# stonkgs/stonkgs

Measured on AMD Instinct MI355X. Metric: text-triple pairs/sec (whole node), seq_len=512 hidden=768, 1/2/4/8 MI355X, higher is better.
Workload: dtype bf16; 1 GPU; STonKGs-150k pretraining step (12L/768h, V=28996, K=175094), per-GPU batch 64, seq 256 text + 256 entity, dropout 0.1, AdamW lr 1e-4; global_batch=64, seq_len=512, parallelism=dp1

## Files before the change

### include/stonk_hip.h

```cpp
#ifndef STONK_HIP_H
#define STONK_HIP_H
#include <stdint.h>
#include "../stonkgs_amd/csrc/stonk_flags.h"

#ifdef __cplusplus
extern "C" {
#endif

#define STONK_OK 0
#define STONK_EINVAL (-1)
#define STONK_ESHAPE (-2)
#define STONK_EALIGN (-3)

int stonk_abi_version(void);

int stonk_gemm_nt_bf16(const void* A, int64_t lda, const void* B, int64_t ldb, void* C, int64_t ldc, int M, int N, int K,
                       int flags, const float* bias, const void* resid, int64_t ldr, void* aux, int64_t ldaux,
                       float alpha, int split_k, const int* m_dev, const int* k_dev, float drop_p, uint32_t seed,
                       int kernel, void* stream);

int stonk_gemm_tn_bf16(const void* dY, int64_t lda, const void* X, int64_t ldb, float* dW, int64_t ldc, float* dbias,
                       int M, int N, int K, float alpha, int split_k, const int* k_dev, void* stream);
int stonk_gemm_tn_bf16_store(const void* dY, int64_t lda, const void* X, int64_t ldb, float* dW, int64_t ldc, float* dbias,
                             int M, int N, int K, float alpha, int split_k, const int* k_dev, void* stream);
int stonk_gemm_tn_bf16_store_sumsq(const void* dY, int64_t lda, const void* X, int64_t ldb, float* dW, int64_t ldc,
                                   float* dbias, int M, int N, int K, float alpha, int split_k, const int* k_dev,
                                   float* tile_sumsq, int64_t n_slots, void* stream);
int64_t stonk_gemm_tn_store_tiles(int M, int N, int K, int split_k);

int stonk_layernorm_fwd(const void* x, const float* gamma, const float* beta, void* y, float* mean, float* rstd,
                        int64_t rows, int H, float eps, int flags, float drop_p, uint32_t seed, void* stream);

int64_t stonk_layernorm_bwd_workspace_floats(int64_t rows, int H);
int stonk_layernorm_bwd(const void* dy, const void* x, const float* mean, const float* rstd, const float* gamma,
                        void* dx, void* dx_drop, float* dgamma, float* dbeta, int64_t rows, int H, int flags,
                        float drop_p_in, uint32_t seed_in, float drop_p_out, uint32_t seed_out, float* partial_ws,
                        int64_t ws_floats, void* stream);
int stonk_layernorm_bwd_reduce(const float* partial_ws, int64_t rows, int H, float* dgamma, float* dbeta, void* stream);

int stonk_joint_embed_ln_fwd(const int64_t* input_ids, const int64_t* token_type_ids, const void* text_hidden,
                             const float* kg_table, const float* pos_emb, const float* type_emb, const float* gamma,
                             const float* beta, void* sum_out, void* y, float* mean, float* rstd, int B, int S,
                             int half, int H, int64_t kg_rows, int type_rows, float eps, int flags, float drop_p,
                             uint32_t seed, int* err_flag, const int* pos_of_row, int64_t n_rows, void* stream);

int stonk_text_embed_ln_fwd(const int64_t* input_ids, int64_t ld_ids, const float* word_emb, const float* pos_emb,
                            const float* type_emb, const float* gamma, const float* beta, void* y, int B, int S, int H,
                            int64_t vocab, float eps, int flags, float drop_p, uint32_t seed, int* err_flag,
                            void* stream);

int stonk_embed_grad(const void* dx, const int64_t* token_type_ids, float* dpos, float* dtype, int B, int S, int H,
                     int type_rows, const int* row_of_pos, void* stream);

int stonk_word_embed_grad(const void* dsum, int64_t ld, const int64_t* input_ids, const int* row_of_pos, float* dword,
                          int64_t ld_w, int64_t vocab, int padding_idx, int B, int S, int H, int* err_flag, void* stream);
// ... 155 lines not shown
```

### stonkgs_amd/_hip.py

```python
from __future__ import annotations

import ctypes as C
import os

_HERE = os.path.dirname(os.path.abspath(__file__))
LIB_PATH = os.environ.get("STONK_HIP_LIB") or os.path.join(_HERE, "csrc", "libstonk_hip.so")

EPI_OUT_BF16 = 0
EPI_OUT_F32 = 1
EPI_OUT_F32_ATOMIC = 2
EPI_OUT_F16 = 3
EPI_BIAS = 1 << 2
EPI_GELU = 1 << 3
EPI_RESID = 1 << 4
EPI_SAVE_PREACT = 1 << 5
EPI_GELU_BWD = 1 << 6
EPI_DROPOUT = 1 << 7
EPI_AUX_GRAD = 1 << 8
GEMM_AUTO, GEMM_TILE128, GEMM_WAVE8, GEMM_WAVE4, GEMM_WAVE4_192, GEMM_DISPATCHED, GEMM_DISPATCHED2 = 0, 1, 2, 3, 4, 5, 6
GEMM_ASM4, GEMM_ASM4_192 = 7, 8
LN_DROPOUT = 1 << 0
LN_DEFER_REDUCE = 1 << 1
SMALL_TANH = 1
SMALL_X_F32 = 16
LOSS_MSE, LOSS_MSE_BROADCAST, LOSS_BCE = 0, 1, 2
OK, EINVAL, ESHAPE, EALIGN = 0, -1, -2, -3
ATTN_BWD_DELTA, ATTN_BWD_DQ, ATTN_BWD_DKV, ATTN_BWD_ALL = 1, 2, 4, 7

_vp, _i32, _i64, _f32, _u32, _f64 = C.c_void_p, C.c_int, C.c_int64, C.c_float, C.c_uint32, C.c_double

_SIGNATURES = {
    "stonk_gemm_nt_bf16": [_vp, _i64, _vp, _i64, _vp, _i64, _i32, _i32, _i32, _i32, _vp, _vp, _i64, _vp, _i64,
                           _f32, _i32, _vp, _vp, _f32, _u32, _i32, _vp],
    "stonk_gemm_tn_bf16": [_vp, _i64, _vp, _i64, _vp, _i64, _vp, _i32, _i32, _i32, _f32, _i32, _vp, _vp],
    "stonk_gemm_tn_bf16_store": [_vp, _i64, _vp, _i64, _vp, _i64, _vp, _i32, _i32, _i32, _f32, _i32, _vp, _vp],
    "stonk_gemm_tn_bf16_store_sumsq": [_vp, _i64, _vp, _i64, _vp, _i64, _vp, _i32, _i32, _i32, _f32, _i32, _vp, _vp, _i64, _vp],
    "stonk_layernorm_fwd": [_vp, _vp, _vp, _vp, _vp, _vp, _i64, _i32, _f32, _i32, _f32, _u32, _vp],
    "stonk_layernorm_bwd": [_vp, _vp, _vp, _vp, _vp, _vp, _vp, _vp, _vp, _i64, _i32, _i32, _f32, _u32, _f32, _u32,
                            _vp, _i64, _vp],
    "stonk_layernorm_bwd_reduce": [_vp, _i64, _i32, _vp, _vp, _vp],
    "stonk_joint_embed_ln_fwd": [_vp, _vp, _vp, _vp, _vp, _vp, _vp, _vp, _vp, _vp, _vp, _vp, _i32, _i32, _i32, _i32,
                                 _i64, _i32, _f32, _i32, _f32, _u32, _vp, _vp, _i64, _vp],
    "stonk_unpad_plan": [_vp, _vp, _vp, _i32, _i32, _i32, _vp, _vp, _vp, _vp, _vp, _vp, _vp, _vp, _i64, _vp],
    "stonk_text_embed_ln_fwd": [_vp, _i64, _vp, _vp, _vp, _vp, _vp, _vp, _i32, _i32, _i32, _i64, _f32, _i32, _f32,
                                _u32, _vp, _vp],
    "stonk_embed_grad": [_vp, _vp, _vp, _vp, _i32, _i32, _i32, _i32, _vp, _vp],
    "stonk_word_embed_grad": [_vp, _i64, _vp, _vp, _vp, _i64, _i64, _i32, _i32, _i32, _i32, _vp, _vp],
    "stonk_input_attribution": [_vp, _i64, _vp, _vp, _vp, _i64, _vp, _f32, _vp, _vp, _vp, _i64, _i32, _i32, _i32, _i32, _vp],
    "stonk_attention_fwd": [_vp, _vp, _vp, _i64, _vp, _vp, _vp, _vp, _i64, _vp, _i32, _i32, _i32, _i32, _f32, _f32, _u32, _vp],
    "stonk_attention_bwd": [_vp, _vp, _vp, _i64, _vp, _vp, _vp, _vp, _i64, _vp, _i64, _vp, _vp, _vp, _vp, _i64, _vp, _i32,
                            _i32, _i32, _i32, _f32, _f32, _u32, _vp],
    "stonk_attention_bwd_phases": [_i32, _vp, _vp, _vp, _i64, _vp, _vp, _vp, _vp, _i64, _vp, _i64, _vp, _vp, _vp, _vp, _i64, _vp,
                                   _i32, _i32, _i32, _i32, _f32, _f32, _u32, _vp],
    "stonk_block_sparse_attention_fwd": [_vp, _vp, _vp, _i64, _vp, _vp, _vp, _vp, _vp, _i64, _vp, _i32, _i32, _i32, _i32, _f32,
                                         _vp, _vp],
    "stonk_block_sparse_attention_bwd": [_vp, _vp, _vp, _i64, _vp, _vp, _vp, _vp, _vp, _vp, _vp, _vp, _i64, _vp, _i64, _vp, _vp,
                                         _vp, _vp, _i64, _vp, _i32, _i32, _i32, _i32, _f32, _vp, _vp],
    "stonk_attention_probs": [_vp, _vp, _i64, _vp, _vp, _vp, _i32, _i32, _i32, _i32, _i32, _f32, _vp],
    "stonk_transpose_bf16": [_vp, _i64, _vp, _i64, _i64, _i32, _vp, _vp, _vp],
    "stonk_transpose_f32_to_bf16": [_vp, _vp, _i64, _i32, _i64, _vp],
    "stonk_transpose_bf16_batched": [_vp, _i32, _i32, _vp],
    "stonk_cast_f32_to_bf16": [_vp, _vp, _i64, _vp],
    "stonk_mlm_mask": [_vp, _vp, _vp, _vp, _i32, _i32, _i32, _i64, _i64, _i64, _i32, _i32, _u32, _vp],
    "stonk_assemble_rows": [_vp, _vp, _vp, _vp, _vp, _i64, _i32, _vp, _vp, _vp, _vp, _i32, _i32, _i32, _i64, _f32, _u32, _vp,
                            _vp],
    "stonk_label_compact": [_vp, _i64, _i32, _i32, _i32, _vp, _vp, _vp, _vp, _vp],
    "stonk_gather_rows_bf16": [_vp, _i64, _vp, _vp, _vp, _i64, _i32, _i64, _vp],
    "stonk_scatter_rows_bf16": [_vp, _i64, _vp, _vp, _vp, _i64, _i32, _vp],
    "stonk_scatter_rows_f32_to_bf16": [_vp, _i64, _vp, _vp, _vp, _i64, _i32, _vp],
# ... 12 lines not shown
    "stonk_sumsq_f32": [_vp, _i64, _vp, _vp, _i64, _vp],
    "stonk_sumsq_f32_plus": [_vp, _i64, _vp, _vp, _i64, _vp, _i64, _vp],
    "stonk_adamw_step": [_vp, _vp, _vp, _vp, _vp, _i64, _f32, _f32, _f32, _f32, _f32, _f32, _f32, _vp, _f32, _f32,
                         _vp, _i32, _i64, _vp],
    "stonk_adamw_step_tiled": [_vp, _vp, _vp, _vp, _vp, _i64, _f32, _f32, _f32, _f32, _f32, _f32, _f32, _vp, _f32, _f32,
                               _vp, _i32, _vp, _i32, _vp, _i32, _i32, _vp, _i32, _i32, _vp],
    "stonk_scale_f32": [_vp, _i64, _f32, _vp],
    "stonk_random_walks": [_vp, _vp, _i64, _vp, _i64, _i64, _i32, _u32, _u32, _u32, _u32, _vp, _i64, _vp],
    "stonk_sgns_step": [_vp, _i64, _i32, _i64, _i64, _i32, _i32, _vp, _vp, _i64, _i32, _i32, _i32, _vp, _vp, _f32, _u32,
                        _vp, _vp],
    "stonk_sample_non_edges": [_vp, _vp, _i64, _i64, _i64, _u32, _vp, _vp, _vp],
    "stonk_linkpred_lossgrad": [_vp, _i64, _i64, _i32, _vp, _vp, _i64, _vp, _f32, _vp, _vp, _vp],
    "stonk_walk_maxpool": [_vp, _i64, _i64, _i32, _vp, _i64, _i64, _i32, _vp, _i64, _vp, _vp],
    "stonk_kgb_train_steps": [_vp, _i64, _i64, _i32, _vp, _i32, _i32, _vp, _i64, _i32, _vp, _vp, _i32, _vp, _vp, _vp, _vp, _vp,
                              _vp, _vp, _vp, _i64, _vp, _f64, _f64, _f64, _f64, _f64, _f32, _u32, _vp],
    "stonk_kgb_predict": [_vp, _i64, _i64, _i32, _vp, _i64, _vp, _vp, _i32, _vp, _vp, _vp, _vp],
    "stonk_transe_step": [_vp, _vp, _i64, _i64, _i32, _vp, _i64, _vp, _i64, _i64, _i32, _i32, _f32, _f32, _u32, _u32, _vp, _vp],
    "stonk_rows_l2_normalize": [_vp, _i64, _i64, _i64, _i32, _vp],
    "stonk_transe_rank": [_vp, _vp, _i64, _i64, _i32, _i32, _vp, _i64, _i32, _vp, _vp, _i64, _vp, _vp, _vp],
    "stonk_comm_unique_id": [_vp],
    "stonk_comm_init": [C.POINTER(C.c_void_p), _i32, _i32, _vp, _i32],
    "stonk_comm_allreduce_async": [_vp, _vp, _i64, _i32, _vp],
    "stonk_comm_reduce_scatter_async": [_vp, _vp, _vp, _i64, _i32, _vp],
    "stonk_comm_allgather_async": [_vp, _vp, _vp, _i64, _i32, _vp],
    "stonk_comm_wait": [_vp, _vp],
    "stonk_comm_destroy": [_vp],
}


class StonkHipError(RuntimeError):
    pass


_lib = None


def lib():
    global _lib
    if _lib is None:
        if not os.path.exists(LIB_PATH):
            raise StonkHipError(
                f"{LIB_PATH} is missing: build it with `make` (or __graft_entry__.build()). "
                "There is no CPU fallback for the STonKGs hot path."
            )
        import torch

        handle = C.CDLL(LIB_PATH)
        missing = [name for name in _SIGNATURES if not hasattr(handle, name)]
        if missing and os.environ.get("STONK_DEV_PARTIAL") == "1":
            for name in missing:
                _SIGNATURES.pop(name)
        elif missing:
            raise StonkHipError(f"{LIB_PATH} does not export {missing}; rebuild with `make`")
        for name, argtypes in _SIGNATURES.items():
            fn = getattr(handle, name)
            fn.argtypes = argtypes
            fn.restype = C.c_int
        handle.stonk_abi_version.argtypes = []
        handle.stonk_abi_version.restype = C.c_int
        handle.stonk_layernorm_bwd_workspace_floats.argtypes = [_i64, _i32]
        handle.stonk_layernorm_bwd_workspace_floats.restype = C.c_int64
        handle.stonk_sumsq_workspace_floats.argtypes = []
        handle.stonk_sumsq_workspace_floats.restype = C.c_int64
        handle.stonk_gemm_tn_store_tiles.argtypes = [_i32, _i32, _i32, _i32]
        handle.stonk_gemm_tn_store_tiles.restype = C.c_int64
        handle.stonk_linkpred_partial_rows.argtypes = []
# ... 36 lines not shown
```

### stonkgs_amd/csrc/gemm_common.h

```cpp
#pragma once
#include <type_traits>

#include "common.h"
#include "stonk_flags.h"

namespace stonk_gemm {

struct GemmArgs {
  const bf16* A;
  const bf16* B;
  void* C;
  const float* bias;
  const bf16* resid;
  bf16* aux;
  const int* m_dev;
  const int* k_dev;
  long lda, ldb, ldc, ldr, ldaux;
  int M, N, K;
  int flags;
  float alpha;
  int split_k;
  uint32_t drop_thr32;
  float drop_scale;
  uint32_t seed;
};

__device__ __forceinline__ int xcd_remap(int b, int n) {
  const int q = n >> 3, r = n & 7, x = b & 7;
  const int base = (x < r) ? x * (q + 1) : r * (q + 1) + (x - r) * q;
  return base + (b >> 3);
}

__device__ __forceinline__ void barrier() { __builtin_amdgcn_s_barrier(); }
template <int N>
__device__ __forceinline__ void wait_vm() {
  static_assert(N >= 0 && N <= 63, "vmcnt is six bits");
  asm volatile("s_waitcnt vmcnt(%0)" ::"n"(N) : "memory");
}
__device__ __forceinline__ void wait_lgkm0() { asm volatile("s_waitcnt lgkmcnt(0)" ::: "memory"); }

struct Work {
  int m0, n0;
  long k_begin;
  int nk;
};

__device__ __forceinline__ int live_count(const int* dev, int cap, int per = 1) {
  if (dev) {
    const int d = (*dev + per - 1) / per;
    cap = d < cap ? d : cap;
  }
  return cap;
}

struct TileRC {
  int rt, ct;
};
__device__ __forceinline__ TileRC tile_split(int tt, int ntm, int ntn) {
  if (ntm >= ntn) {
// ... 139 lines not shown
```

### stonkgs_amd/csrc/gemm_tn.hip

```cpp
#include <cstdlib>

#include "gemm_common.h"

int stonk_gemm256_tn_launch(const stonk_gemm::GemmArgs& a, hipStream_t st);
int stonk_gemm_tn_a4_launch(const stonk_gemm::GemmArgs& a, hipStream_t st);
int stonk_gemm_tn_a4_store_launch(const stonk_gemm::GemmArgs& a, hipStream_t st);
int stonk_gemm_tn_a4_store_sumsq_launch(const stonk_gemm::GemmArgs& a, hipStream_t st);

namespace {

constexpr int BM = 128, BN = 128, BK = 64;
constexpr int TILE_BYTES = BK * 256;
constexpr int STAGE_BYTES = 2 * TILE_BYTES;
constexpr int TN_LDS = 2 * STAGE_BYTES;

using stonk_gemm::live_count;
using stonk_gemm::tile_split;
using stonk_gemm::xcd_remap;

struct TnArgs {
  const bf16* A;
  const bf16* B;
  float* C;
  float* bias;
  const int* k_dev;
  long lda, ldb, ldc;
  int M, N, K;
  float alpha;
  int split_k;
  float* tile_sumsq;
};

__device__ __forceinline__ int row_swz(int row) { return ((row & 3) << 2) | ((row >> 2) & 3); }

typedef __attribute__((address_space(3))) bf16x4 lds_bf16x4;

template <bool STORE, bool SUMSQ>
__device__ __forceinline__ void gemm_tn_body(const TnArgs& p) {
  extern __shared__ __attribute__((aligned(16))) char smem[];
  const int tid = threadIdx.x;
// ... 118 lines not shown
        if constexpr (STORE) p.bias[m] = accb[i][r] * p.alpha;
        else atomicAdd(p.bias + m, accb[i][r] * p.alpha);
      }
    }
    if constexpr (SUMSQ) {
      float sr[4];
#pragma unroll
      for (int r = 0; r < 4; ++r) sr[r] = (sq[r][0] + sq[r][1]) + (sq[r][2] + sq[r][3]);
      ss += (sr[0] + sr[1]) + (sr[2] + sr[3]);
    }
  }
  if constexpr (SUMSQ) {
    float* part = (float*)smem;
    ss = wave_sum(ss);
    __syncthreads();
    if (lane == 0) part[wave] = ss;
    __syncthreads();
    if (tid == 0) p.tile_sumsq[rt * ntn + ct] = ((part[0] + part[1]) + part[2]) + part[3];
  }
}

template <bool STORE>
__global__ __launch_bounds__(256, 2) void gemm_tn_kernel(const TnArgs p) {
  gemm_tn_body<STORE, false>(p);
}
__global__ __launch_bounds__(256, 2) void gemm_tn_store_sumsq_kernel(const TnArgs p) { gemm_tn_body<true, true>(p); }

}

static long gemm_tn_store_tiles(int M, int N, int split_k) {
  return split_k <= 0 ? (long)((M + 255) / 256) * ((N + 255) / 256) : (long)(M / BM) * (N / BN);
}

static int gemm_tn_route(const void* dY, int64_t lda, const void* X, int64_t ldb, float* dW, int64_t ldc, float* dbias,
                         int M, int N, int K, float alpha, int split_k, const int* k_dev, void* stream, bool store,
                         float* tile_sumsq = nullptr, int64_t n_slots = 0, bool dry = false) {
  STONK_CHECK_ARG(dY && X && dW, STONK_EINVAL);
  STONK_CHECK_ARG(M > 0 && N > 0 && K > 0 && M % BM == 0 && N % BN == 0, STONK_ESHAPE);
  STONK_CHECK_ARG(lda % 8 == 0 && ldb % 8 == 0, STONK_EALIGN);
  STONK_CHECK_ARG((uintptr_t)dY % 16 == 0 && (uintptr_t)X % 16 == 0, STONK_EALIGN);
  if (store) {
    STONK_CHECK_ARG(ldc >= N && (long)M * ldc * 4 < (1L << 31), STONK_ESHAPE);
    STONK_CHECK_ARG((uintptr_t)dW % 4 == 0 && (uintptr_t)dbias % 4 == 0, STONK_EALIGN);
  }
  if (split_k <= 0) {
    STONK_CHECK_ARG(M >= 256 && N >= 256, STONK_ESHAPE);
    STONK_CHECK_ARG(lda % 64 == 0 && ldb % 64 == 0 && lda < (1L << 23) && ldb < (1L << 23), STONK_ESHAPE);
    STONK_CHECK_ARG(split_k >= -1024, STONK_ESHAPE);
    stonk_gemm::GemmArgs g = {};
    g.A = (const bf16*)dY; g.B = (const bf16*)X; g.C = dW; g.bias = dbias; g.k_dev = k_dev;
    g.lda = lda; g.ldb = ldb; g.ldc = ldc; g.M = M; g.N = N; g.K = K; g.alpha = alpha;
    const int nk = (K + BK - 1) / BK;
    const long tiles = (long)((M + 255) / 256) * ((N + 255) / 256);
    const long cus = split_k <= -16 ? -split_k : 256;
    long sk = tiles >= cus ? 1 : cus / tiles;
    if (sk > nk / 8) sk = nk / 8 > 0 ? nk / 8 : 1;
    g.split_k = (int)sk;
    g.flags = (int)cus;
    if (store) {
      STONK_CHECK_ARG(sk == 1 && split_k != -1, STONK_ESHAPE);
      STONK_CHECK_ARG(!dbias || N <= 256, STONK_ESHAPE);
      if (dry) return STONK_OK;
      if (!tile_sumsq) return stonk_gemm_tn_a4_store_launch(g, (hipStream_t)stream);
      STONK_CHECK_ARG(n_slots >= gemm_tn_store_tiles(M, N, split_k), STONK_EINVAL);
      g.aux = (bf16*)tile_sumsq;
      return stonk_gemm_tn_a4_store_sumsq_launch(g, (hipStream_t)stream);
    }
    return split_k == -1 ? stonk_gemm256_tn_launch(g, (hipStream_t)stream) : stonk_gemm_tn_a4_launch(g, (hipStream_t)stream);
  }
  TnArgs a;
  a.A = (const bf16*)dY; a.B = (const bf16*)X; a.C = dW; a.bias = dbias; a.k_dev = k_dev;
  a.lda = lda; a.ldb = ldb; a.ldc = ldc; a.M = M; a.N = N; a.K = K; a.alpha = alpha;
  const int nk = (K + BK - 1) / BK;
  a.split_k = split_k < nk ? split_k : nk;
  const long tiles = (long)(M / BM) * (N / BN) * a.split_k;
  a.tile_sumsq = tile_sumsq;
  if (store) {
    STONK_CHECK_ARG(a.split_k == 1, STONK_ESHAPE);
    if (dry) return STONK_OK;
    if (!tile_sumsq) return stonk_gemm::launch_with_lds<gemm_tn_kernel<true>, TN_LDS>(a, (int)tiles, 256, (hipStream_t)stream);
    STONK_CHECK_ARG(n_slots >= tiles, STONK_EINVAL);
    return stonk_gemm::launch_with_lds<gemm_tn_store_sumsq_kernel, TN_LDS>(a, (int)tiles, 256, (hipStream_t)stream);
  }
  return stonk_gemm::launch_with_lds<gemm_tn_kernel<false>, TN_LDS>(a, (int)tiles, 256, (hipStream_t)stream);
}

extern "C" int stonk_gemm_tn_bf16(const void* dY, int64_t lda, const void* X, int64_t ldb, float* dW, int64_t ldc,
                                  float* dbias, int M, int N, int K, float alpha, int split_k, const int* k_dev,
                                  void* stream) {
  return gemm_tn_route(dY, lda, X, ldb, dW, ldc, dbias, M, N, K, alpha, split_k, k_dev, stream, false);
}

extern "C" int stonk_gemm_tn_bf16_store(const void* dY, int64_t lda, const void* X, int64_t ldb, float* dW, int64_t ldc,
                                        float* dbias, int M, int N, int K, float alpha, int split_k, const int* k_dev,
                                        void* stream) {
  return gemm_tn_route(dY, lda, X, ldb, dW, ldc, dbias, M, N, K, alpha, split_k, k_dev, stream, true);
}

extern "C" int stonk_gemm_tn_bf16_store_sumsq(const void* dY, int64_t lda, const void* X, int64_t ldb, float* dW,
                                              int64_t ldc, float* dbias, int M, int N, int K, float alpha, int split_k,
                                              const int* k_dev, float* tile_sumsq, int64_t n_slots, void* stream) {
  STONK_CHECK_ARG(tile_sumsq && n_slots >= 0, STONK_EINVAL);
  STONK_CHECK_ARG((uintptr_t)tile_sumsq % 4 == 0, STONK_EALIGN);
  return gemm_tn_route(dY, lda, X, ldb, dW, ldc, dbias, M, N, K, alpha, split_k, k_dev, stream, true, tile_sumsq, n_slots);
}

extern "C" int64_t stonk_gemm_tn_store_tiles(int M, int N, int K, int split_k) {
  static const int dummy = 0;
  const void* q = (const void*)(((uintptr_t)&dummy + 4096) & ~(uintptr_t)15);
  const int rc = gemm_tn_route(q, M, q, N, (float*)q, N, nullptr, M, N, K, 1.f, split_k, nullptr, nullptr, true, nullptr, 0, true);
  return rc != STONK_OK ? rc : gemm_tn_store_tiles(M, N, split_k);
}
```

### stonkgs_amd/csrc/gemm_tn_a4.hip

```cpp
#include "gemm_common.h"
#ifndef STONK_TN_A4_STORE
#define STONK_TN_A4_STORE 0
#endif
#if STONK_TN_A4_STORE == 2
#define STONK_TN_A4_KERNEL gemm_tn_a4_store_sumsq_kernel
#define STONK_TN_A4_LAUNCH stonk_gemm_tn_a4_store_sumsq_launch
#elif STONK_TN_A4_STORE
#define STONK_TN_A4_KERNEL gemm_tn_a4_store_kernel
#define STONK_TN_A4_LAUNCH stonk_gemm_tn_a4_store_launch
#else
#define STONK_TN_A4_KERNEL gemm_tn_a4_kernel
#define STONK_TN_A4_LAUNCH stonk_gemm_tn_a4_launch
#endif
#ifndef STONK_A4_LOOP_INC
#define STONK_A4_LOOP_INC "gemm_a4_loop.inc"
#endif
#include STONK_A4_LOOP_INC

using namespace stonk_gemm;

namespace {

constexpr int BM = 256, BN = 256, BK = 64;
constexpr int IMG_BYTES = BK * 512;
constexpr int IMG_LDS = 4 * IMG_BYTES;
constexpr int LDS_BYTES = IMG_LDS + (STONK_TN_A4_STORE == 2 ? 16 : 0);

typedef __attribute__((ext_vector_type(4))) int i32x4;
typedef __attribute__((ext_vector_type(4))) unsigned u32x4;

struct Cursor {
  i32x4 srd;
  int rem_lo, rem_hi;
};

__global__ __launch_bounds__(256, 1) void STONK_TN_A4_KERNEL(const GemmArgs p) {
  extern __shared__ __attribute__((aligned(16))) char smem[];
  const int tid = threadIdx.x;
  const int lane = tid & 63;
  const int wave = __builtin_amdgcn_readfirstlane(tid >> 6);
  const int wr = wave >> 1, wc = wave & 1;

  const int M = p.M, N = p.N;
  const int Kact = live_count(p.k_dev, p.K);
  const int ntm = (M + BM - 1) / BM, ntn = (N + BN - 1) / BN;
  const int nk_total = (Kact + BK - 1) / BK;
  int nk_per = (nk_total + p.split_k - 1) / p.split_k;
  nk_per += nk_per & 1;
  const int per_split = ntm * ntn;
  const int total = per_split * p.split_k;
  const int G = gridDim.x;
#if STONK_TN_A4_STORE
  if (nk_total == 0) {
    const int ldc0 = (int)p.ldc;
    for (int w = blockIdx.x; w < total; w += G) {
      const int rt = ntm >= ntn ? w / ntn : w % ntm, ct = ntm >= ntn ? w % ntn : w / ntm;
      const int n = ct * BN + tid;
      for (int r = 0; r < BM; ++r) {
        const int m = rt * BM + r;
        if (m < M && n < N) ((float*)p.C)[(long)m * ldc0 + n] = 0.f;
      }
      if (p.bias && ct == 0 && rt * BM + tid < M) ((float*)p.bias)[rt * BM + tid] = 0.f;
#if STONK_TN_A4_STORE == 2
      if (tid == 0) ((float*)p.aux)[rt * ntn + ct] = 0.f;
#endif
    }
    return;
  }
#endif

  auto get_work = [&](int w, Work& o) -> bool {
    if (w >= total) return false;
    int idx = w;
    {
      const int r = w / G, b = w - r * G;
      const int x = b & 7, base = G >> 3, rem = G & 7;
      const int cand = r * G + x * base + (x < rem ? x : rem) + (b >> 3);
      if ((r + 1) * G <= total) idx = cand;
    }
    const int ks = idx / per_split;
    const int tt = idx - ks * per_split;
    const TileRC t = tile_split(tt, ntm, ntn);
    o.m0 = t.rt * BM;
    o.n0 = t.ct * BN;
// ... 14 lines not shown
    voffA[q] = row * lda2 + c;
    voffB[q] = row * ldb2 + c;
  }
  const unsigned lds0 = (unsigned)(size_t)(__attribute__((address_space(3))) char*)smem;
  const int m0a = (int)lds0 + wave * 8192;
  const int m0b = (int)lds0 + 2 * IMG_BYTES + wave * 8192;
  int taA[8], taB[8];
  {
    const int g = lane >> 4, q = (lane & 15) >> 2, pq = lane & 3;
    const int f = q | ((g & 1) << 2);
    const int rowb = (8 * g + q) * 512 + pq * 8;
#pragma unroll
    for (int i = 0; i < 8; ++i) {
      taA[i] = (int)lds0 + rowb + ((8 * wr + (i ^ f)) << 5);
      taB[i] = (int)lds0 + 2 * IMG_BYTES + rowb + ((8 * wc + (i ^ f)) << 5);
    }
  }
  const u32x4 ones = {0x3F803F80u, 0x3F803F80u, 0x3F803F80u, 0x3F803F80u};

  auto cursor_of = [&](const Work& w, Cursor& a, Cursor& b) {
    const unsigned long pa = (unsigned long)p.A + (unsigned long)((w.k_begin * p.lda + w.m0) * 2);
    const unsigned long pb = (unsigned long)p.B + (unsigned long)((w.k_begin * p.ldb + w.n0) * 2);
    const long ra = ((long)Kact - w.k_begin) * lda2 - (long)w.m0 * 2, rb = ((long)Kact - w.k_begin) * ldb2 - (long)w.n0 * 2;
    auto clamp = [](long r) -> int { return (int)(unsigned)(r < 0 ? 0 : (r > 0xFFFFF000L ? 0xFFFFF000L : r)); };
    a.srd = (i32x4){(int)(unsigned)pa, (int)((pa >> 32) & 0xffff), clamp(ra), 0x00020000};
    b.srd = (i32x4){(int)(unsigned)pb, (int)((pb >> 32) & 0xffff), clamp(rb), 0x00020000};
    a.rem_lo = (int)(unsigned)ra;
    a.rem_hi = (int)(ra >> 32);
    b.rem_lo = (int)(unsigned)rb;
    b.rem_hi = (int)(rb >> 32);
  };

  Work cw, nw;
  int cwi = blockIdx.x;
  if (!get_work(cwi, cw)) return;
  if (cw.nk <= 0 && !next_live_work(get_work, cwi, G, cw)) return;
  Cursor ca, cb;
  cursor_of(cw, ca, cb);
  const int stepa = BK * lda2, stepb = BK * ldb2;

#define STONK_TN_A4_DMA_OPERANDS \
  STONK_A4_VOFF_IN(voffA, voffB), [m0a] "s"(m0a), [m0b] "s"(m0b), [stepa] "s"(stepa), [stepb] "s"(stepb)

  asm volatile(STONK_TN_A4_PROLOGUE
               : "+{s[36:39]}"(ca.srd), "+{s[40:43]}"(cb.srd), [ralo] "+s"(ca.rem_lo), [rahi] "+s"(ca.rem_hi),
                 [rblo] "+s"(cb.rem_lo), [rbhi] "+s"(cb.rem_hi)
               : STONK_TN_A4_DMA_OPERANDS
               : "m0", "scc", "s48", "memory");

  const bool want_bias = p.bias != nullptr;
  const int r16 = lane & 15, qq = lane >> 4;

  for (;;) {
    int nwi = cwi;
    const bool more = next_live_work(get_work, nwi, G, nw);
    Cursor na, nb;
    cursor_of(more ? nw : cw, na, nb);
    f32x16 acc[16];
    f32x4 bacc[8];
#pragma unroll
    for (int i = 0; i < 8; ++i) bacc[i] = (f32x4){0.f, 0.f, 0.f, 0.f};
    int rem = cw.nk >> 1;
    const int ct = cw.n0 / BN;
    const int kt0 = (int)(cw.k_begin / BK);
    int bph = want_bias ? ((kt0 - ct) % ntn + ntn) % ntn : 1;
    const int ntn_s = want_bias ? ntn : 0x7fffffff;
    asm volatile(STONK_TN_A4_TILE
// ... 69 lines not shown
      }
#endif
#if STONK_TN_A4_STORE
      if (want_bias && wc == 0 && ct == 0) {
        const int boff = r16 == 0 ? 0 : 0x40000000;
#pragma unroll
        for (int e = 0; e < 4; ++e)
          __builtin_amdgcn_raw_buffer_store_b32(__float_as_uint(bacc[i][e] * p.alpha), rBias, (wm0 + 16 * i + 4 * qq + e) * 4 + boff, 0, 0);
      }
#else
      if (want_bias && wc == 0) {
        const int boff = r16 == 0 ? 0 : 0x40000000;
#pragma unroll
        for (int e = 0; e < 4; ++e)
          __builtin_amdgcn_raw_ptr_buffer_atomic_fadd_f32(bacc[i][e] * p.alpha, rBias, (wm0 + 16 * i + 4 * qq + e) * 4 + boff, 0, 0);
      }
#endif
    }
#if STONK_TN_A4_STORE == 2
    {
      volatile float* part = (volatile float*)(smem + IMG_LDS);
      ss = wave_sum(ss);
      if (lane == 0) part[wave] = ss;
      asm volatile("s_waitcnt lgkmcnt(0)\n\ts_barrier" ::: "memory");
      if (tid == 0) ((float*)p.aux)[(cw.m0 / BM) * ntn + cw.n0 / BN] = ((part[0] + part[1]) + part[2]) + part[3];
    }
#endif
    if (!more) break;
    cwi = nwi;
    cw = nw;
  }
  asm volatile("s_waitcnt vmcnt(0)" ::: "memory");
#undef STONK_TN_A4_DMA_OPERANDS
}

}

int STONK_TN_A4_LAUNCH(const GemmArgs& a, hipStream_t st) {
  const int n_cu = cu_count();
  if (n_cu <= 0) return (int)hipGetLastError();
  const long tiles = (long)((a.M + BM - 1) / BM) * ((a.N + BN - 1) / BN) * a.split_k;
  const int cap = (a.flags > 0 && a.flags < n_cu) ? a.flags : n_cu;
  const int grid = (int)(tiles < cap ? tiles : cap);
  return launch_with_lds<STONK_TN_A4_KERNEL, LDS_BYTES>(a, grid, 256, st);
}
```

### stonkgs_amd/engine.py

```python
from __future__ import annotations

import collections
import contextlib
import dataclasses
import math
import os
import struct
import time
from typing import Callable, Dict, Optional

import torch

from . import _hip as hip
from .config import STonKGsConfig
from .params import FlatStore, pad128

BF16, F32, I32 = torch.bfloat16, torch.float32, torch.int32

ERR_BITS = {1: "entity id outside the KG table (the reference raises KeyError, stonkgs_model.py:185)",
            2: "token_type_id outside [0, type_vocab_size)", 4: "text token id outside the LM vocabulary",
            8: "MLM/ELM label outside the decoder's class range", 16: "NSP label outside [0, 2)"}

Decoder = collections.namedtuple("Decoder", "name label_key weight classes offset")

# ... 97 lines not shown
        self.saved = None
        self.seed_base = 0x5710
        self.overlap_wgrad = True
        self.comm_overlap = False
        self.kernel_for: Dict[str, int] = {}
        self.f16_logits = True
        self.unpad = True
        self.prune_last_ffn = True
        self.prune_last_attn = True
        self.next_input_ids: Optional[torch.Tensor] = None
        self._prefetch: Optional[dict] = None
        self._bb_stream: Optional[torch.cuda.Stream] = None
        self._pref_par = 0
        self.rows_executed = [0, 0, 0, 0, 0, 0, 0]
        self._plan_host: Optional[torch.Tensor] = None
        self._wstream: Optional[torch.cuda.Stream] = None
        self._opt_stream: Optional[torch.cuda.Stream] = None
        self._params_ready: Optional[torch.cuda.Event] = None
        self.marks: Optional[list] = None
        self._wgrad_done: Dict[int, torch.cuda.Event] = {}
        self._wt_desc = None
        self._adamw_tables = None
        self.store_names: tuple = ()
        self.store_first = False
        self.grad_stale: set = set()
        self.store_log = collections.deque(maxlen=64)
        self.norm_from_epilogue = True
        self.store_sumsq = False
        self.sumsq_valid: set = set()
        self._sumsq_tiles: Dict[str, int] = {}
        self._sumsq_buf: Optional[torch.Tensor] = None
        self._inputs_only = False
        self.tn_cus = 160
        self.roctx = bool(os.environ.get("STONK_ROCTX"))
        self.tn_min_k = 16384
        self.tn_min_tiles = 36

    def buf(self, name: str, shape, dtype=BF16, zero=False) -> torch.Tensor:
        n = 1
        for d in shape:
            n *= d
        t = self.ws.get(name)
        if t is None or t.numel() < n or t.dtype != dtype:
            t = (torch.zeros if zero else torch.empty)(max(n, 1), dtype=dtype, device=self.device)
            self.ws[name] = t
        return t[:n].view(shape)

    @contextlib.contextmanager
    def optimizer_stream(self, enabled: bool = True):
        if not enabled:
            yield
            return
        with self._fork("_opt_stream") as stream:
            yield
            ev = torch.cuda.Event()
            ev.record(stream)
        self._params_ready = ev

    @contextlib.contextmanager
    def _fork(self, attr: str):
        side = getattr(self, attr)
        if side is None:
            side = torch.cuda.Stream(device=self.device)
            setattr(self, attr, side)
        side.wait_stream(torch.cuda.current_stream())
        with torch.cuda.stream(side):
# ... 81 lines not shown
        if tiles >= self.tn_min_tiles and K >= self.tn_min_k and M % 256 == 0 and N % 256 == 0:
            return -self.tn_cus if side_stream else 0
        return max(1, min(32, 480 // tiles, K // 64))

    def wgrad(self, dy, x, dW, db, M_out, N_in, T, k_dev=None, alpha=1.0, name=None):
        if self._inputs_only:
            return
        self.sumsq_valid.discard(name)
        side = self.overlap_wgrad
        split = self._split_k(M_out, N_in, T, side)
        with (self._fork("_wstream") if side else contextlib.nullcontext()), \
                self._timed("tn_a4" if split <= 0 else "tn", M_out, N_in, T, None, k_dev):
            args = (dy.data_ptr(), dy.stride(0), x.data_ptr(), x.stride(0), dW.data_ptr(), dW.stride(0), hip.ptr(db), M_out,
                    N_in, T, alpha, split, hip.ptr(k_dev), hip.stream_ptr())
            can_store = db is None and dW.stride(0) >= N_in and M_out * dW.stride(0) * 4 < 1 << 31
            if name is not None and self.store_first and name in self.store_names and can_store:
                slots = self._sumsq_slots(name, M_out, N_in, T, split) if self.store_sumsq and self.norm_from_epilogue else None
                if slots is None:
                    rc = hip.lib().stonk_gemm_tn_bf16_store(*args)
                else:
                    rc = hip.lib().stonk_gemm_tn_bf16_store_sumsq(*args[:-1], slots.data_ptr(), slots.numel(), args[-1])
                self.store_log.append((name, rc))
                if rc == hip.OK:
                    self.grad_stale.discard(name)
                    if slots is not None:
                        self.sumsq_valid.add(name)
                    return
                if rc != hip.ESHAPE:
                    hip.check(rc, "stonk_gemm_tn_bf16_store")
            if name in self.grad_stale:
                dW.zero_()
                self.grad_stale.discard(name)
            hip.call("stonk_gemm_tn_bf16", *args)

    def _sumsq_slots(self, name, M, N, K, split) -> Optional[torch.Tensor]:
        n = int(hip.lib().stonk_gemm_tn_store_tiles(M, N, K, split))
        if n <= 0:
            return None
        at = self.store_names.index(name)
        if self._sumsq_tiles.get(name) != n:
            self._sumsq_tiles[name] = n
            self.sumsq_valid.difference_update(self.store_names[at + 1:])
        total = sum(self._sumsq_tiles.values())
        if self._sumsq_buf is None or self._sumsq_buf.numel() < total:
            self._sumsq_buf = torch.zeros(max(total, 16384), dtype=F32, device=self.device)
            self.sumsq_valid.clear()
        first = sum(self._sumsq_tiles.get(k, 0) for k in self.store_names[:at])
        return self._sumsq_buf[first:first + n]

    def take_wgrad_sumsq(self):
        ok = bool(self.store_names) and self.sumsq_valid == set(self.store_names)
        self.sumsq_valid.clear()
        if not ok:
            return None
        total = sum(self._sumsq_tiles[k] for k in self.store_names)
        return sorted(self.P.span(k) for k in self.store_names), self._sumsq_buf[:total]

    def _gather_rows(self, src, rd_rows, cnt, dst, cap) -> None:
        H = self.cfg.hidden_size
        hip.call("stonk_gather_rows_bf16", src.data_ptr(), H, rd_rows.data_ptr(), cnt.data_ptr(), dst.data_ptr(), H, H, cap,
                 hip.stream_ptr())

    def _scatter_rows_into_zeros(self, src, rd_rows, cnt, dst, T) -> None:
        H = self.cfg.hidden_size
        dst[:T].zero_()
        hip.call("stonk_scatter_rows_bf16", src.data_ptr(), H, rd_rows.data_ptr(), cnt.data_ptr(), dst.data_ptr(), H, H,
# ... 134 lines not shown
                  resid=hf, drop_p=p_hid, seed=self.seed(lidx, 3), kernel=self._kernel("ffn_down"))
        y = self.buf(f"{prefix}.y" if save is not None else f"tmp.y{lidx & 1}", (cap, H))
        st2 = self.buf(f"{tag}.st2", (2, cap), F32)
        hip.call("stonk_layernorm_fwd", s2.data_ptr(), f(prefix + ".output.LayerNorm.weight").data_ptr(),
                 f(prefix + ".output.LayerNorm.bias").data_ptr(), y.data_ptr(), st2[0].data_ptr(), st2[1].data_ptr(), Tf,
                 H, cfg.layer_norm_eps, 0, 0.0, 0, st)
        if save is not None:
            save[prefix] = dict(x=x, qkv=qkv, ctx=ctx, ctx_in=a_in, lse=lse, s1=s1, h1=hf, st1=st1, g=g, u=u, s2=s2, st2=st2)
        return y

    def layer_bwd(self, prefix: str, dy, L: Rows, p_hid, p_att, lidx, sv, last: bool = False):
        cfg = self.cfg
        H, I, NH = cfg.hidden_size, cfg.intermediate_size, cfg.num_attention_heads
        B, seq, T, mask, cu = L.B, L.S, L.T, L.mask, L.cu
        rd = L.rd if last else None
        cap = B * seq
        st = hip.stream_ptr()
        P = self.P
        g_ = P.grad_view
        f = P.view
        wt = P.wt
        par = lidx & 1
        ev = self._wgrad_done.pop(par, None)
        if ev is not None:
            torch.cuda.current_stream().wait_event(ev)
        ds2 = self.buf(f"b.ds2.{par}", (cap, H))
        df = self.buf(f"b.df.{par}", (cap, H)) if p_hid > 0 else None
        Tf = T if rd is None else rd.T
        self.ln_bwd(dy, sv["s2"], sv["st2"][0], sv["st2"][1], f(prefix + ".output.LayerNorm.weight"), ds2, df,
                    g_(prefix + ".output.LayerNorm.weight"), g_(prefix + ".output.LayerNorm.bias"), Tf, H, 0, 0.0, 0, p_hid,
                    self.seed(lidx, 3))
        if df is None:
            df = ds2
        self.wgrad(df, sv["g"], g_(prefix + ".output.dense.weight"), g_(prefix + ".output.dense.bias"), H, I, Tf)
        du = self.buf(f"b.du.{par}", (cap, I))
        self.gemm(df, wt[prefix + ".output.dense.weight"], du, Tf, I, H, flags=hip.EPI_GELU_BWD | hip.EPI_AUX_GRAD,
                  aux=sv["u"], kernel=self._kernel("dgrad_gelu", True))
        self.wgrad(du, sv["h1"], g_(prefix + ".intermediate.dense.weight"), g_(prefix + ".intermediate.dense.bias"), I, H,
                   Tf)
        qattn = rd is not None and rd.attn
        Ta = Tf if qattn else T
        dh1 = self.buf("b.dh1", (cap, H))
        gathered = rd is not None and not qattn
        dh1f = self.buf("b.dh1rd", (cap, H)) if gathered else dh1
        self.gemm(du, wt[prefix + ".intermediate.dense.weight"], dh1f, Tf, H, I, flags=hip.EPI_RESID, resid=ds2,
                  kernel=self._kernel("dgrad_resid", True))
        if gathered:
            self._scatter_rows_into_zeros(dh1f, rd.rows, rd.cnt, dh1, T)
        ds1 = self.buf(f"b.ds1.{par}", (cap, H))
        da = self.buf(f"b.da.{par}", (cap, H)) if p_hid > 0 else None
        self.ln_bwd(dh1, sv["s1"], sv["st1"][0], sv["st1"][1], f(prefix + ".attention.output.LayerNorm.weight"), ds1, da,
                    g_(prefix + ".attention.output.LayerNorm.weight"), g_(prefix + ".attention.output.LayerNorm.bias"), Ta, H, 0,
                    0.0, 0, p_hid, self.seed(lidx, 2))
        if da is None:
            da = ds1
        self.wgrad(da, sv["ctx_in"], g_(prefix + ".attention.output.dense.weight"),
                   g_(prefix + ".attention.output.dense.bias"), H, H, Ta)
        dctx = self.buf("b.dctx", (cap, H))
        dctxa = self.buf("b.dctxrd", (cap, H)) if qattn else dctx
        self.gemm(da, wt[prefix + ".attention.output.dense.weight"], dctxa, Ta, H, H,
                  kernel=self._kernel("dgrad_attn_out", True))
        if qattn:
            ds1rd, ds1 = ds1, self.buf("b.ds1full", (cap, H))
            self._scatter_rows_into_zeros(dctxa, rd.rows, rd.cnt, dctx, T)
            self._scatter_rows_into_zeros(ds1rd, rd.rows, rd.cnt, ds1, T)
        qkv = sv["qkv"]
        dqkv = self.buf(f"b.dqkv.{par}", (cap, 3 * H))
        delta = self.buf("b.delta", (B, NH, seq), F32)
        qoff = rd.offsets if qattn else None
        if qattn:
            dqkv[:T, :H].zero_()
        aargs = (qkv.data_ptr(), qkv.data_ptr() + 2 * H, qkv.data_ptr() + 4 * H, 3 * H, hip.ptr(mask), hip.ptr(cu),
                 hip.ptr(qoff), sv["ctx"].data_ptr(), H, dctx.data_ptr(), H, sv["lse"].data_ptr(), delta.data_ptr(),
                 dqkv.data_ptr(), dqkv.data_ptr() + 2 * H, 3 * H, dqkv.data_ptr() + 4 * H, B, NH, seq, 64,
                 1.0 / math.sqrt(64.0), p_att, self.seed(lidx, 1))
        hip.call("stonk_attention_bwd", *aargs, st)
        self.wgrad(dqkv, sv["x"], g_(prefix + ".attention.self.qkv.weight"), g_(prefix + ".attention.self.qkv.bias"),
                   3 * H, H, T)
        dx = self.buf(f"b.dx{lidx & 1}", (cap, H))
        self.gemm(dqkv, wt[prefix + ".attention.self.qkv.weight"], dx, T, H, 3 * H, flags=hip.EPI_RESID, resid=ds1,
                  kernel=self._kernel("dgrad_resid", True))
        if self._wstream is not None and self.overlap_wgrad:
            done = torch.cuda.Event()
            done.record(self._wstream)
            self._wgrad_done[par] = done
        return dx

    def backbone_fwd(self, input_ids, ld_ids, B, seq, training: bool, mask=None):
        cfg = self.cfg
        H = cfg.hidden_size
        p_hid = cfg.hidden_dropout_prob if training else 0.0
        p_att = cfg.attention_probs_dropout_prob if training else 0.0
        f = self.BB.view
        x = self.buf("bb.x", (B * seq, H))
        hip.call("stonk_text_embed_ln_fwd", input_ids.data_ptr(), ld_ids,
                 f("lm_backbone.embeddings.word_embeddings.weight").data_ptr(),
                 f("lm_backbone.embeddings.position_embeddings.weight").data_ptr(),
                 f("lm_backbone.embeddings.token_type_embeddings.weight").data_ptr(),
                 f("lm_backbone.embeddings.LayerNorm.weight").data_ptr(),
                 f("lm_backbone.embeddings.LayerNorm.bias").data_ptr(), x.data_ptr(), B, seq, H, cfg.vocab_size,
                 cfg.layer_norm_eps, hip.LN_DROPOUT if p_hid > 0 else 0, p_hid, self.seed(100, 0), self.err.data_ptr(),
                 hip.stream_ptr())
        L = padded_rows(B, seq, mask)
        for i in range(self.n_bb):
            x = self.layer_fwd(self.BB, f"lm_backbone.encoder.layer.{i}", x, L, p_hid, p_att, 101 + i, None)
        return x

    def prefetch_backbone(self, input_ids, training: bool) -> None:
        cfg = self.cfg
        H, S, half = cfg.hidden_size, cfg.max_position_embeddings, cfg.half_length
        B = input_ids.shape[0]
# ... 618 lines not shown
```

Before: 2476 pairs/s.

## Group attention-output and QKV weight-gradient GEMMs into one persistent launch

Adds a grouped TN GEMM kernel that runs up to four weight-gradient problems in a single launch, assigning blocks to problems by offset and choosing a shared split-K that fits within the CU budget. The attention output and QKV wgrads are deferred and launched together on the wgrad stream instead of as two separate launches. The aim is to fill the GPU better with these small GEMMs and cut launch overhead. The cost is that the attention-output wgrad now starts later, and any shape the grouped kernel rejects falls back to the per-GEMM path.

```diff
diff --git a/include/stonk_hip.h b/include/stonk_hip.h
--- a/include/stonk_hip.h
+++ b/include/stonk_hip.h
@@ -21,6 +21,16 @@
 
 int stonk_gemm_tn_bf16(const void* dY, int64_t lda, const void* X, int64_t ldb, float* dW, int64_t ldc, float* dbias,
                        int M, int N, int K, float alpha, int split_k, const int* k_dev, void* stream);
+typedef struct StonkTnProblem {
+  const void* dY; int64_t lda;
+  const void* X; int64_t ldb;
+  float* dW; int64_t ldc;
+  float* dbias;
+  const int* k_dev;
+  int M, N, K;
+  float alpha;
+} StonkTnProblem;
+int stonk_gemm_tn_bf16_group(const StonkTnProblem* problems, int n, int cu_cap, void* stream);
 int stonk_gemm_tn_bf16_store(const void* dY, int64_t lda, const void* X, int64_t ldb, float* dW, int64_t ldc, float* dbias,
                              int M, int N, int K, float alpha, int split_k, const int* k_dev, void* stream);
 int stonk_gemm_tn_bf16_store_sumsq(const void* dY, int64_t lda, const void* X, int64_t ldb, float* dW, int64_t ldc,
diff --git a/stonkgs_amd/_hip.py b/stonkgs_amd/_hip.py
--- a/stonkgs_amd/_hip.py
+++ b/stonkgs_amd/_hip.py
@@ -35,6 +35,7 @@
     "stonk_gemm_tn_bf16": [_vp, _i64, _vp, _i64, _vp, _i64, _vp, _i32, _i32, _i32, _f32, _i32, _vp, _vp],
     "stonk_gemm_tn_bf16_store": [_vp, _i64, _vp, _i64, _vp, _i64, _vp, _i32, _i32, _i32, _f32, _i32, _vp, _vp],
     "stonk_gemm_tn_bf16_store_sumsq": [_vp, _i64, _vp, _i64, _vp, _i64, _vp, _i32, _i32, _i32, _f32, _i32, _vp, _vp, _i64, _vp],
+    "stonk_gemm_tn_bf16_group": [_vp, _i32, _i32, _vp],
     "stonk_layernorm_fwd": [_vp, _vp, _vp, _vp, _vp, _vp, _i64, _i32, _f32, _i32, _f32, _u32, _vp],
     "stonk_layernorm_bwd": [_vp, _vp, _vp, _vp, _vp, _vp, _vp, _vp, _vp, _i64, _i32, _i32, _f32, _u32, _f32, _u32,
                             _vp, _i64, _vp],
@@ -113,6 +114,19 @@
     pass
 
 
+class TnProblem(C.Structure):
+    _fields_ = [("dY", _vp), ("lda", _i64), ("X", _vp), ("ldb", _i64), ("dW", _vp), ("ldc", _i64), ("dbias", _vp),
+                ("k_dev", _vp), ("M", _i32), ("N", _i32), ("K", _i32), ("alpha", _f32)]
+
+
+def tn_problems(members):
+    arr = (TnProblem * len(members))()
+    for q, (dY, lda, X, ldb, dW, ldc, dbias, M, N, K, alpha, k_dev) in zip(arr, members):
+        q.dY, q.lda, q.X, q.ldb, q.dW, q.ldc, q.dbias, q.k_dev = dY, lda, X, ldb, dW, ldc, dbias, k_dev
+        q.M, q.N, q.K, q.alpha = M, N, K, alpha
+    return arr
+
+
 _lib = None
 
 
diff --git a/stonkgs_amd/csrc/gemm_common.h b/stonkgs_amd/csrc/gemm_common.h
--- a/stonkgs_amd/csrc/gemm_common.h
+++ b/stonkgs_amd/csrc/gemm_common.h
@@ -25,6 +25,13 @@
   uint32_t seed;
 };
 
+struct TnGroupArgs {
+  static constexpr int MAX = 4;
+  GemmArgs prob[MAX];
+  int first[MAX], items[MAX];
+  int n;
+};
+
 __device__ __forceinline__ int xcd_remap(int b, int n) {
   const int q = n >> 3, r = n & 7, x = b & 7;
   const int base = (x < r) ? x * (q + 1) : r * (q + 1) + (x - r) * q;
diff --git a/stonkgs_amd/csrc/gemm_tn.hip b/stonkgs_amd/csrc/gemm_tn.hip
--- a/stonkgs_amd/csrc/gemm_tn.hip
+++ b/stonkgs_amd/csrc/gemm_tn.hip
@@ -1,11 +1,13 @@
 #include <cstdlib>
 
 #include "gemm_common.h"
+#include "stonk_hip.h"
 
 int stonk_gemm256_tn_launch(const stonk_gemm::GemmArgs& a, hipStream_t st);
 int stonk_gemm_tn_a4_launch(const stonk_gemm::GemmArgs& a, hipStream_t st);
 int stonk_gemm_tn_a4_store_launch(const stonk_gemm::GemmArgs& a, hipStream_t st);
 int stonk_gemm_tn_a4_store_sumsq_launch(const stonk_gemm::GemmArgs& a, hipStream_t st);
+int stonk_gemm_tn_a4_group_launch(const stonk_gemm::TnGroupArgs& g, int grid, hipStream_t st);
 
 namespace {
 
@@ -190,6 +192,13 @@
   return split_k <= 0 ? (long)((M + 255) / 256) * ((N + 255) / 256) : (long)(M / BM) * (N / BN);
 }
 
+static int tn_a4_shape_status(int64_t lda, int64_t ldb, int64_t ldc, int M, int N) {
+  STONK_CHECK_ARG(M >= 256 && N >= 256, STONK_ESHAPE);
+  STONK_CHECK_ARG(lda % 64 == 0 && ldb % 64 == 0 && lda < (1L << 23) && ldb < (1L << 23), STONK_ESHAPE);
+  STONK_CHECK_ARG(ldc >= N && (long)M * ldc * 4 < (1L << 31), STONK_ESHAPE);
+  return STONK_OK;
+}
+
 static int gemm_tn_route(const void* dY, int64_t lda, const void* X, int64_t ldb, float* dW, int64_t ldc, float* dbias,
                          int M, int N, int K, float alpha, int split_k, const int* k_dev, void* stream, bool store,
                          float* tile_sumsq = nullptr, int64_t n_slots = 0, bool dry = false) {
@@ -202,8 +211,7 @@
     STONK_CHECK_ARG((uintptr_t)dW % 4 == 0 && (uintptr_t)dbias % 4 == 0, STONK_EALIGN);
   }
   if (split_k <= 0) {
-    STONK_CHECK_ARG(M >= 256 && N >= 256, STONK_ESHAPE);
-    STONK_CHECK_ARG(lda % 64 == 0 && ldb % 64 == 0 && lda < (1L << 23) && ldb < (1L << 23), STONK_ESHAPE);
+    if (const int rc = tn_a4_shape_status(lda, ldb, ldc, M, N)) return rc;
     STONK_CHECK_ARG(split_k >= -1024, STONK_ESHAPE);
     stonk_gemm::GemmArgs g = {};
     g.A = (const bf16*)dY; g.B = (const bf16*)X; g.C = dW; g.bias = dbias; g.k_dev = k_dev;
@@ -249,6 +257,46 @@
   return gemm_tn_route(dY, lda, X, ldb, dW, ldc, dbias, M, N, K, alpha, split_k, k_dev, stream, false);
 }
 
+extern "C" int stonk_gemm_tn_bf16_group(const StonkTnProblem* problems, int n, int cu_cap, void* stream) {
+  using stonk_gemm::TnGroupArgs;
+  STONK_CHECK_ARG(problems && n > 0 && cu_cap >= 0, STONK_EINVAL);
+  STONK_CHECK_ARG(n <= TnGroupArgs::MAX && cu_cap <= 1024, STONK_ESHAPE);
+  TnGroupArgs g = {};
+  long tiles_all = 0, sk = 1L << 30;
+  for (int i = 0; i < n; ++i) {
+    const StonkTnProblem& q = problems[i];
+    STONK_CHECK_ARG(q.dY && q.X && q.dW, STONK_EINVAL);
+    STONK_CHECK_ARG(q.M > 0 && q.N > 0 && q.K > 0 && q.M % 256 == 0 && q.N % 256 == 0, STONK_ESHAPE);
+    STONK_CHECK_ARG(q.lda % 8 == 0 && q.ldb % 8 == 0, STONK_EALIGN);
+    STONK_CHECK_ARG((uintptr_t)q.dY % 16 == 0 && (uintptr_t)q.X % 16 == 0, STONK_EALIGN);
+    STONK_CHECK_ARG((uintptr_t)q.dW % 4 == 0 && (uintptr_t)q.dbias % 4 == 0, STONK_EALIGN);
+    if (const int rc = tn_a4_shape_status(q.lda, q.ldb, q.ldc, q.M, q.N)) return rc;
+    stonk_gemm::GemmArgs& a = g.prob[i];
+    a.A = (const bf16*)q.dY; a.B = (const bf16*)q.X; a.C = q.dW; a.bias = q.dbias; a.k_dev = q.k_dev;
+    a.lda = q.lda; a.ldb = q.ldb; a.ldc = q.ldc; a.M = q.M; a.N = q.N; a.K = q.K; a.alpha = q.alpha;
+    tiles_all += (long)(q.M / 256) * (q.N / 256);
+    const long by_k = ((q.K + BK - 1) / BK) / 8;
+    sk = by_k < sk ? by_k : sk;
+  }
+  long cap = cu_cap;
+  if (cap == 0) {
+    cap = stonk_gemm::cu_count();
+    if (cap <= 0) return (int)hipGetLastError();
+  }
+  STONK_CHECK_ARG(tiles_all <= cap, STONK_ESHAPE);
+  sk = sk < cap / tiles_all ? sk : cap / tiles_all;
+  sk = sk > 0 ? sk : 1;
+  int at = 0;
+  for (int i = 0; i < n; ++i) {
+    g.prob[i].split_k = (int)sk;
+    g.items[i] = (int)((long)(g.prob[i].M / 256) * (g.prob[i].N / 256) * sk);
+    g.first[i] = at;
+    at += i + 1 < n ? (g.items[i] + 7) & ~7 : g.items[i];
+  }
+  g.n = n;
+  return stonk_gemm_tn_a4_group_launch(g, at, (hipStream_t)stream);
+}
+
 extern "C" int stonk_gemm_tn_bf16_store(const void* dY, int64_t lda, const void* X, int64_t ldb, float* dW, int64_t ldc,
                                         float* dbias, int M, int N, int K, float alpha, int split_k, const int* k_dev,
                                         void* stream) {
diff --git a/stonkgs_amd/csrc/gemm_tn_a4.hip b/stonkgs_amd/csrc/gemm_tn_a4.hip
--- a/stonkgs_amd/csrc/gemm_tn_a4.hip
+++ b/stonkgs_amd/csrc/gemm_tn_a4.hip
@@ -2,7 +2,13 @@
 #ifndef STONK_TN_A4_STORE
 #define STONK_TN_A4_STORE 0
 #endif
-#if STONK_TN_A4_STORE == 2
+#ifndef STONK_TN_A4_GROUP
+#define STONK_TN_A4_GROUP 0
+#endif
+#if STONK_TN_A4_GROUP
+#define STONK_TN_A4_KERNEL gemm_tn_a4_group_kernel
+#define STONK_TN_A4_LAUNCH stonk_gemm_tn_a4_group_launch
+#elif STONK_TN_A4_STORE == 2
 #define STONK_TN_A4_KERNEL gemm_tn_a4_store_sumsq_kernel
 #define STONK_TN_A4_LAUNCH stonk_gemm_tn_a4_store_sumsq_launch
 #elif STONK_TN_A4_STORE
@@ -34,7 +40,20 @@
   int rem_lo, rem_hi;
 };
 
+#if STONK_TN_A4_GROUP
+__global__ __launch_bounds__(256, 1) void STONK_TN_A4_KERNEL(const TnGroupArgs g) {
+  int pi = 0;
+#pragma unroll
+  for (int i = 1; i < TnGroupArgs::MAX; ++i) pi = (i < g.n && (int)blockIdx.x >= g.first[i]) ? i : pi;
+  const GemmArgs& p = g.prob[pi];
+  const int bid = (int)blockIdx.x - g.first[pi];
+  const int G = g.items[pi];
+  if (bid >= G) return;
+#define STONK_TN_A4_BID bid
+#else
 __global__ __launch_bounds__(256, 1) void STONK_TN_A4_KERNEL(const GemmArgs p) {
+#define STONK_TN_A4_BID blockIdx.x
+#endif
   extern __shared__ __attribute__((aligned(16))) char smem[];
   const int tid = threadIdx.x;
   const int lane = tid & 63;
@@ -49,7 +68,9 @@
   nk_per += nk_per & 1;
   const int per_split = ntm * ntn;
   const int total = per_split * p.split_k;
+#if !STONK_TN_A4_GROUP
   const int G = gridDim.x;
+#endif
 #if STONK_TN_A4_STORE
   if (nk_total == 0) {
     const int ldc0 = (int)p.ldc;
@@ -130,7 +151,7 @@
   };
 
   Work cw, nw;
-  int cwi = blockIdx.x;
+  int cwi = STONK_TN_A4_BID;
   if (!get_work(cwi, cw)) return;
   if (cw.nk <= 0 && !next_live_work(get_work, cwi, G, cw)) return;
   Cursor ca, cb;
@@ -266,10 +287,16 @@
   }
   asm volatile("s_waitcnt vmcnt(0)" ::: "memory");
 #undef STONK_TN_A4_DMA_OPERANDS
+#undef STONK_TN_A4_BID
 }
 
 }
 
+#if STONK_TN_A4_GROUP
+int STONK_TN_A4_LAUNCH(const TnGroupArgs& g, int grid, hipStream_t st) {
+  return launch_with_lds<STONK_TN_A4_KERNEL, LDS_BYTES>(g, grid, 256, st);
+}
+#else
 int STONK_TN_A4_LAUNCH(const GemmArgs& a, hipStream_t st) {
   const int n_cu = cu_count();
   if (n_cu <= 0) return (int)hipGetLastError();
@@ -278,3 +305,4 @@
   const int grid = (int)(tiles < cap ? tiles : cap);
   return launch_with_lds<STONK_TN_A4_KERNEL, LDS_BYTES>(a, grid, 256, st);
 }
+#endif
diff --git a/stonkgs_amd/csrc/gemm_tn_a4_group.hip b/stonkgs_amd/csrc/gemm_tn_a4_group.hip
--- /dev/null
+++ b/stonkgs_amd/csrc/gemm_tn_a4_group.hip
@@ -0,0 +1,2 @@
+#define STONK_TN_A4_GROUP 1
+#include "gemm_tn_a4.hip"
diff --git a/stonkgs_amd/engine.py b/stonkgs_amd/engine.py
--- a/stonkgs_amd/engine.py
+++ b/stonkgs_amd/engine.py
@@ -153,6 +153,8 @@
         self._sumsq_buf: Optional[torch.Tensor] = None
         self._inputs_only = False
         self.tn_cus = 160
+        self.wgrad_groups: frozenset = frozenset({"attn"})
+        self.group_log = collections.deque(maxlen=64)
         self.roctx = bool(os.environ.get("STONK_ROCTX"))
         self.tn_min_k = 16384
         self.tn_min_tiles = 36
@@ -300,6 +302,26 @@
                 dW.zero_()
                 self.grad_stale.discard(name)
             hip.call("stonk_gemm_tn_bf16", *args)
+
+    def _groupable(self, kind: str, shapes) -> bool:
+        if kind not in self.wgrad_groups or not self.overlap_wgrad or self._inputs_only:
+            return False
+        return len({T for _, _, T in shapes}) == 1 and all(self._split_k(M, N, T, True) <= 0 for M, N, T in shapes)
+
+    def wgrad_group(self, members) -> None:
+        T = members[0][6]
+        probs = hip.tn_problems([(dy.data_ptr(), dy.stride(0), x.data_ptr(), x.stride(0), dW.data_ptr(), dW.stride(0), hip.ptr(db),
+                                  M, N, T, 1.0, 0) for dy, x, dW, db, M, N, T in members])
+        with self._fork("_wstream"), self._timed("tn_a4", sum(m[4] * m[5] for m in members), 1, T):
+            rc = hip.lib().stonk_gemm_tn_bf16_group(probs, len(members), self.tn_cus, hip.stream_ptr())
+        self.group_log.append((len(members), rc))
+        if rc == hip.ESHAPE:
+            if self.gemm_timer is not None:
+                self.gemm_timer.records.pop()
+            for m in members:
+                self.wgrad(*m)
+            return
+        hip.check(rc, "stonk_gemm_tn_bf16_group")
 
     def _sumsq_slots(self, name, M, N, K, split) -> Optional[torch.Tensor]:
         n = int(hip.lib().stonk_gemm_tn_store_tiles(M, N, K, split))
@@ -500,12 +522,18 @@
                     self.seed(lidx, 3))
         if df is None:
             df = ds2
-        self.wgrad(df, sv["g"], g_(prefix + ".output.dense.weight"), g_(prefix + ".output.dense.bias"), H, I, Tf)
+        w_down = (df, sv["g"], g_(prefix + ".output.dense.weight"), g_(prefix + ".output.dense.bias"), H, I, Tf)
+        group_ffn = self._groupable("ffn", [(H, I, Tf), (I, H, Tf)])
+        if not group_ffn:
+            self.wgrad(*w_down)
         du = self.buf(f"b.du.{par}", (cap, I))
         self.gemm(df, wt[prefix + ".output.dense.weight"], du, Tf, I, H, flags=hip.EPI_GELU_BWD | hip.EPI_AUX_GRAD,
                   aux=sv["u"], kernel=self._kernel("dgrad_gelu", True))
-        self.wgrad(du, sv["h1"], g_(prefix + ".intermediate.dense.weight"), g_(prefix + ".intermediate.dense.bias"), I, H,
-                   Tf)
+        w_up = (du, sv["h1"], g_(prefix + ".intermediate.dense.weight"), g_(prefix + ".intermediate.dense.bias"), I, H, Tf)
+        if group_ffn:
+            self.wgrad_group([w_down, w_up])
+        else:
+            self.wgrad(*w_up)
         qattn = rd is not None and rd.attn
         Ta = Tf if qattn else T
         dh1 = self.buf("b.dh1", (cap, H))
@@ -522,8 +550,11 @@
                     0.0, 0, p_hid, self.seed(lidx, 2))
         if da is None:
             da = ds1
-        self.wgrad(da, sv["ctx_in"], g_(prefix + ".attention.output.dense.weight"),
-                   g_(prefix + ".attention.output.dense.bias"), H, H, Ta)
+        w_out = (da, sv["ctx_in"], g_(prefix + ".attention.output.dense.weight"),
+                 g_(prefix + ".attention.output.dense.bias"), H, H, Ta)
+        group_attn = self._groupable("attn", [(3 * H, H, T), (H, H, Ta)])
+        if not group_attn:
+            self.wgrad(*w_out)
         dctx = self.buf("b.dctx", (cap, H))
         dctxa = self.buf("b.dctxrd", (cap, H)) if qattn else dctx
         self.gemm(da, wt[prefix + ".attention.output.dense.weight"], dctxa, Ta, H, H,
@@ -543,8 +574,11 @@
                  dqkv.data_ptr(), dqkv.data_ptr() + 2 * H, 3 * H, dqkv.data_ptr() + 4 * H, B, NH, seq, 64,
                  1.0 / math.sqrt(64.0), p_att, self.seed(lidx, 1))
         hip.call("stonk_attention_bwd", *aargs, st)
-        self.wgrad(dqkv, sv["x"], g_(prefix + ".attention.self.qkv.weight"), g_(prefix + ".attention.self.qkv.bias"),
-                   3 * H, H, T)
+        w_qkv = (dqkv, sv["x"], g_(prefix + ".attention.self.qkv.weight"), g_(prefix + ".attention.self.qkv.bias"), 3 * H, H, T)
+        if group_attn:
+            self.wgrad_group([w_qkv, w_out])
+        else:
+            self.wgrad(*w_qkv)
         dx = self.buf(f"b.dx{lidx & 1}", (cap, H))
         self.gemm(dqkv, wt[prefix + ".attention.self.qkv.weight"], dx, T, H, 3 * H, flags=hip.EPI_RESID, resid=ds1,
                   kernel=self._kernel("dgrad_resid", True))
```

Result: faster. 2502 pairs/s (median of 6 runs) (+1.1%).
